# OSU-NLP-Group/saev

Hardware: AMD Instinct MI355X
Metric: activations/sec (train step), d_in=1024 x32 k=32 (higher is better)
Workload: dtype f32 (encoder: fp16 MFMA first pass with a rigorous error margin, survivors recomputed exactly in fp32; all else fp32)

## Files before the change

saev_amd/csrc/ctx_forward.hip:

```cpp
#include "ctx.h"

extern "C" {


int saev_normalize_w_dec(saev_ctx* c, void* stream) {
    if (!c) return SAEV_INVALID_ARG;
    REQUIRE(c, c->params, SAEV_NOT_BOUND, "parameters not bound");
    if (!c->cfg.normalize_w_dec) return SAEV_OK;
    HIPCHK(c, launch_normalize_rows(c->params + c->off_W_dec, c->cfg.d_sae, c->cfg.d_model, (hipStream_t)stream));
    return SAEV_OK;
}

static bool bind_x_sources(saev_ctx* c, const float* x, int n, bool allow_borrow) {
    saev_ctx* l = c->leader;
    const bool borrow = allow_borrow && l != nullptr && l->xprep_x == x && l->xprep_n == n && l->xprep_serial != c->leader_serial_seen;
    saev_ctx* src = borrow ? l : c;
    c->upper_c = src->upper; c->mu_c = src->mu; c->xnorm_c = src->xnorm; c->xabs_c = src->xabs_part; c->xs_c = src->xs;
    c->borrow_streamed = borrow && l->fwd_streamed && l->mu_keep != nullptr;
    if (c->borrow_streamed) c->mu_c = l->mu_keep;
    c->fwd_step = c->fwd_slices && (src == c || src->fwd_slices);
    c->xS_c = c->fwd_step ? src->xS : nullptr;
    if (borrow) c->leader_serial_seen = l->xprep_serial;
    return borrow;
}
// ... 86 lines not shown
        if (predicted) { a.heur_z = c->heur_state; a.tau_max = c->tau_max; }
        a.refresh_first = 8;
        a.refresh_every = a.ngroups > 32 ? 1 : 2;
        HIPCHK(c, launch_encode_f16x3(a, epi, s));
        return SAEV_OK;
    }
    EncodeArgs a{};
    a.x = x;
    a.W_enc = c->params + c->off_W_enc;
    a.b_enc = c->params + c->off_b_enc;
    a.n_rows = n;
    a.D = c->cfg.d_model;
    a.S = c->cfg.d_sae;
    a.s_splits = encoder_splits(n, a.S, encode_gemm_tile_rows(), encode_gemm_tile_latents(), 512);
    a.h_out = h_out;
    a.ngroups = c->cfg.top_k <= 32 ? 32 : 64;
    a.gmax = c->gmax;
    a.gmax_stride = c->gmax_stride;
    a.cand_cnt = c->cand_cnt;
    a.cand_val = c->cand_val;
    a.cand_idx = c->cand_idx;
    a.cand_cap = CAND_CAP; a.cand_stride = CAND_STRIDE;
    a.enable_flag = flag;
    a.enable_when = when;
    HIPCHK(c, launch_encode_gemm(a, epi, s));
    return SAEV_OK;
}

int saev_encode_dense(saev_ctx* c, const float* x, int32_t n, float* h_out, void* stream) {
    if (!c) return SAEV_INVALID_ARG;
    REQUIRE(c, c->params, SAEV_NOT_BOUND, "parameters not bound");
    REQUIRE(c, x && h_out && n > 0, SAEV_INVALID_ARG, "saev_encode_dense: bad arguments");
    REQUIRE(c, n <= c->cfg.max_batch || c->cfg.encoder_mode == SAEV_ENCODER_F32, SAEV_INVALID_ARG,
            "saev_encode_dense: n_rows > max_batch");
    bind_x_sources(c, x, n, false);
    c->xprep_x = nullptr;
    if (c->relu_train && c->cfg.encoder_mode == SAEV_ENCODER_F16X3) {
        hipStream_t s = (hipStream_t)stream;
        HIPCHK(c, hipMemsetAsync(c->rt_scales + 8, 0, sizeof(float), s));
        HIPCHK(c, launch_absmax(x, (long)n * c->cfg.d_model, c->rt_scales + 8, s));
        int rc = prepare_dense_scaled(c, x, n, c->rt_scales + 8, c->rt_scales + 10, s);
        if (rc != SAEV_OK) return rc;
        return run_encoder(c, x, n, EPI_DENSE, h_out, nullptr, 0, s, false, c->rt_scales + 10);
    }
    if (c->cfg.encoder_mode != SAEV_ENCODER_F16R) {
        int rc = prepare_encoder(c, x, n, nullptr, (hipStream_t)stream);
        if (rc != SAEV_OK) return rc;
    }
    return run_encoder(c, x, n, EPI_DENSE, h_out, nullptr, 0, (hipStream_t)stream);
}

int saev_topk_dense(saev_ctx* c, const float* h, int32_t n, int32_t k, const int32_t* mask, int32_t* idx_out,
                    float* val_out, void* stream) {
    if (!c) return SAEV_INVALID_ARG;
    REQUIRE(c, h && idx_out && val_out && n > 0 && k > 0, SAEV_INVALID_ARG, "saev_topk_dense: bad arguments");
    REQUIRE(c, k <= c->cfg.d_sae, SAEV_INVALID_ARG, "saev_topk_dense: k > d_sae");
    SelectDenseArgs a{};
    a.h = h; a.n_rows = n; a.S = c->cfg.d_sae; a.k = k; a.mask = mask;
    a.idx_out = idx_out; a.val_out = val_out; a.out_stride = k;
    HIPCHK(c, launch_select_dense(a, (hipStream_t)stream));
    return SAEV_OK;
}

static int encode_topk_impl(saev_ctx* c, const float* x, int n, int32_t* idx_out, float* val_out,
                            const int32_t* pre_flag, hipStream_t s, const float* xmax_dev = nullptr, bool x_borrowed = false) {
    const int K = c->cfg.top_k;
    int32_t* need_dense = c->flags + 1;
    const bool f16r_mode = c->cfg.encoder_mode == SAEV_ENCODER_F16R;
    const bool predict_mode = fused_supported(c->cfg) && c->cfg.bound_mode != 0 && c->cfg.encoder_mode != SAEV_ENCODER_F32 &&
                              f16_ngroups(c) == 32;
    const bool one_launch_pre = fused_supported(c->cfg) && !predict_mode;
    if (c->follow_stream) {
        HIPCHK(c, launch_follower_scales(c->leader->xside_keep, c->wmax_prev, scl(c), const_cast<int32_t*>(pre_flag), 1, s));
    } else if (!c->stream_step) {
        int rc0 = prepare_encoder(c, x, n, const_cast<int32_t*>(pre_flag), s, xmax_dev, x_borrowed, one_launch_pre);
        if (rc0 != SAEV_OK) return rc0;
        rc0 = wait_wenc(c, s);
        if (rc0 != SAEV_OK) return rc0;
    }
    if (fused_supported(c->cfg)) {
        const int ng = c->cfg.encoder_mode == SAEV_ENCODER_F32 ? (c->cfg.top_k <= 32 ? 32 : 64) : f16_ngroups(c);
        const bool f16r = c->cfg.encoder_mode == SAEV_ENCODER_F16R;
        auto select_stage = [&](const int32_t* flag, int when, int32_t* bad, const int32_t* tau_max, int32_t* ovf = nullptr,
                                const int32_t* first_flag = nullptr) -> int {
            SelectCandArgs sc{};
            sc.cand_cnt = c->cand_cnt; sc.cand_val = c->cand_val; sc.cand_idx = c->cand_idx;
            sc.cand_cap = CAND_CAP; sc.cand_stride = CAND_STRIDE; sc.n_rows = n; sc.k = K;
            sc.idx_out = idx_out; sc.val_out = val_out; sc.out_stride = K;
            sc.enable_flag = first_flag ? first_flag : flag; sc.enable_when = when;
            sc.tau_max = tau_max; sc.invalid = bad; sc.ovf = ovf;
            if (f16r) {
                sc.row_margin = c->row_margin; sc.x = x; sc.W_encT = c->dW_encT; sc.b_enc = c->params + c->off_b_enc;
                sc.D = c->cfg.d_model; sc.refine_overflow = bad;
                sc.surv_idx = c->surv_idx; sc.surv_val = c->surv_val; sc.surv_cnt = c->surv_cnt;
                if (c->fwd_step) { sc.surv_rng = c->surv_rng; sc.lat_range = c->rs_lat_range; sc.n_ranges = c->rs_n_ranges; }
                HIPCHK(c, launch_select_cand(sc, s));
                sc.enable_flag = flag; sc.ovf = nullptr;
                if (c->fwd_step) {
                    RefineSlicesArgs rs{};
                    rs.surv_idx = c->surv_idx; rs.surv_cnt = c->surv_cnt; rs.surv_val = c->surv_val; rs.surv_rng = c->surv_rng;
                    rs.xS = c->xS_c; rs.WeS = c->stream_ok ? c->WeS : c->dW_encT; rs.b_enc = sc.b_enc; rs.part = c->rs_part;
                    rs.n_rows = n; rs.S = c->cfg.d_sae; rs.D = c->cfg.d_model;
                    rs.lat_range = c->rs_lat_range; rs.n_ranges = c->rs_n_ranges;
                    rs.enable_flag = flag; rs.enable_when = when;
                    HIPCHK(c, launch_refine_slices(rs, s));
                    sc.sum_part = c->rs_part; sc.sum_bias = sc.b_enc; sc.sum_n = c->cfg.d_model / RS_SLICE; sc.sum_plane = (size_t)n * REFINE_CAP;
                } else {
                    HIPCHK(c, launch_refine_exact(sc, s));
                }
                sc.row_margin = nullptr; sc.tau_max = nullptr;
                sc.cand_cnt = c->surv_cnt; sc.cand_val = c->surv_val; sc.cand_idx = c->surv_idx; sc.cand_cap = REFINE_CAP; sc.cand_stride = REFINE_CAP;
            }
            HIPCHK(c, launch_select_cand(sc, s));
            return SAEV_OK;
        };
        const bool predict = c->cfg.bound_mode != 0 && ng == 32 && c->cfg.encoder_mode != SAEV_ENCODER_F32;
        int32_t *bad1 = c->flags + 9, *run2 = c->flags + 10, *gate = c->flags + 11;
        if (predict) {
            HIPCHK(c, launch_heur_gate(c->heur_state, pre_flag, gate, s));
            HIPCHK(c, launch_encoder_init(c->cand_cnt, n, c->gmax, 0, s, c->tau_max));
            timing_begin(c, s);
            int rc = run_encoder(c, x, n, EPI_TOPK, nullptr, gate, 0, s, true);
            if (rc != SAEV_OK) return rc;
            timing_end(c, s);
            HIPCHK(c, launch_overflow_check(c->cand_cnt, n, CAND_CAP, gate, bad1, c->flags + 2, c->flags + 3, s, need_dense,
                                            nullptr, c->heur_state + 3, nullptr, pre_flag));
            rc = select_stage(bad1, 0, bad1, c->tau_max);
            if (rc != SAEV_OK) return rc;
            HIPCHK(c, launch_heur_update(c->heur_state, bad1, c->heur_state + 3, K, gate, s));
            HIPCHK(c, launch_encoder_init(c->cand_cnt, n, c->gmax, ng * c->gmax_stride, s, nullptr, bad1, 1));
            rc = run_encoder(c, x, n, EPI_TOPK, nullptr, bad1, 1, s);
            if (rc != SAEV_OK) return rc;
            HIPCHK(c, launch_overflow_check(c->cand_cnt, n, CAND_CAP, pre_flag, need_dense, c->flags + 2, c->flags + 3, s, need_dense,
                                            run2, nullptr, bad1));
            rc = select_stage(run2, 1, need_dense, nullptr);
            if (rc != SAEV_OK) return rc;
        } else {
            const int S_ = c->cfg.d_sae;
            if (c->stream_step) {
                const int D_ = c->cfg.d_model;
                XprepArgs xp{};
                xp.x = c->gather_pool != nullptr ? c->gather_pool : x; xp.rows = c->gather_rows; xp.x_out = c->gather_pool != nullptr ? const_cast<float*>(x) : nullptr;
                xp.n = n; xp.D = D_; xp.nks = D_ / 32; xp.n_pad = c->MB_pad; xp.scales = scl(c); xp.mu = c->mu; xp.xs = c->xs; xp.xS = c->xS;
                xp.xn_part = c->xn_part; xp.col_part = c->colsum_partials; xp.amax_part = c->amax_part; xp.cmax_part = c->cmax_part;
                xp.W_enc = c->params + c->off_W_enc; xp.WeS = c->WeS; xp.b_enc = c->params + c->off_b_enc; xp.b_seen = c->b_seen;
                xp.S = S_; xp.salt = ++c->stale_salt; xp.stale = c->flags + 12;
                if (!c->followers.empty()) { xp.mu_keep = c->mu_keep; xp.xside_keep = c->xside_keep; }
                HIPCHK(c, launch_xprep(xp, s));
                PreEncode2Args pe{};
                pe.cand_cnt = c->cand_cnt; pe.n_rows = n; pe.gmax = c->gmax; pe.n_gmax = ng * c->gmax_stride;
                pe.xn_part = c->xn_part; pe.nks = D_ / 32; pe.n_pad = c->MB_pad; pe.D = D_;
                pe.wg_part = c->wnorm_scratch; pe.n_part = (S_ + 255) / 256; pe.scales = scl(c); pe.scales_next = scl_next(c);
                pe.pre_flag = const_cast<int32_t*>(pre_flag); pe.wmax_prev = c->wmax_prev; pe.margin = c->row_margin; pe.xnorm = c->xnorm;
                pe.flags1 = c->flags + 1; pe.col_part = c->colsum_partials; pe.n_rowblk = (n + 255) / 256; pe.mu = c->mu;
                pe.inv_n = 1.0f / (float)n; pe.update_mu = c->train_fused ? 1 : 0;
                pe.amax_part = c->amax_part; pe.cmax_part = c->cmax_part; pe.n_img = ((n + 255) / 256) * (D_ / 32);
                pe.upper = c->upper; pe.stats = c->stats; pe.stale = c->flags + 12; pe.stale_host = c->stale_dev;
                pe.xside_keep = c->followers.empty() ? nullptr : c->xside_keep;
                HIPCHK(c, launch_pre_encode2(pe, s));
                if (c->train_fused) c->mu_serial++;
            } else
            HIPCHK(c, launch_pre_encode(c->cand_cnt, n, c->gmax, ng * c->gmax_stride, f16r_mode ? c->xnorm_c : nullptr, c->cfg.d_model,
                                        c->wnorm_scratch, (S_ + 255) / 256, f16r_mode ? scl(c) : nullptr, const_cast<int32_t*>(pre_flag),
                                        c->wmax_prev, c->row_margin, c->flags + 1, s));
            timing_begin(c, s);
            int rc = run_encoder(c, x, n, EPI_TOPK, nullptr, pre_flag, 0, s);
            if (rc != SAEV_OK) return rc;
            timing_end(c, s);
            rc = select_stage(need_dense, 0, need_dense, nullptr, c->flags + 1, pre_flag);
            if (rc != SAEV_OK) return rc;
        }
    } else {
        HIPCHK(c, launch_init_i32(need_dense, 1, 1, s));
        HIPCHK(c, hipMemsetAsync(c->flags + 2, 0, 2 * sizeof(int32_t), s));
        timing_begin(c, s);
        timing_end(c, s);
    }
    int rc = run_encoder(c, x, n, EPI_DENSE, c->h_dense, need_dense, 1, s);
    if (rc != SAEV_OK) return rc;
    SelectDenseArgs sd{};
    sd.h = c->h_dense; sd.n_rows = n; sd.S = c->cfg.d_sae; sd.k = K;
    sd.idx_out = idx_out; sd.val_out = val_out; sd.out_stride = K;
    sd.enable_flag = need_dense; sd.enable_when = 1;
    if (fused_supported(c->cfg)) sd.walk_grid = 4 * 256;
    HIPCHK(c, launch_select_dense(sd, s));
    return SAEV_OK;
}

int saev_encode_topk(saev_ctx* c, const float* x, int32_t n, int32_t* idx_out, float* val_out, void* stream) {
    if (!c) return SAEV_INVALID_ARG;
    REQUIRE(c, c->cfg.activation == SAEV_ACT_TOPK, SAEV_UNSUPPORTED,
            "saev_encode_topk: a TopK context only (ReLU: saev_encode_relu, BatchTopK: saev_encode_batch_topk)");
    REQUIRE(c, c->params, SAEV_NOT_BOUND, "parameters not bound");
    REQUIRE(c, x && idx_out && val_out && n > 0 && n <= c->cfg.max_batch, SAEV_INVALID_ARG,
            "saev_encode_topk: bad arguments (n_rows must be in 1..max_batch)");
    hipStream_t s = (hipStream_t)stream;
    HIPCHK(c, hipMemsetAsync(c->flags, 0, sizeof(int32_t), s));
    bind_x_sources(c, x, n, false);
    c->xprep_x = nullptr;
    c->stream_step = false;
    c->follow_stream = false;
    return encode_topk_impl(c, x, n, idx_out, val_out, c->flags, s);
}

int saev_scatter_dense(saev_ctx* c, const int32_t* idx, const float* val, int32_t n, int32_t k, float* f_out,
                       void* stream) {
    if (!c) return SAEV_INVALID_ARG;
    REQUIRE(c, idx && val && f_out && n > 0 && k > 0, SAEV_INVALID_ARG, "saev_scatter_dense: bad arguments");
    HIPCHK(c, launch_scatter_dense(idx, val, n, k, k, c->cfg.d_sae, f_out, (hipStream_t)stream));
    return SAEV_OK;
// ... 308 lines not shown
```

saev_amd/csrc/kernels.h:

```cpp
#pragma once
#include <hip/hip_runtime.h>
#include <stdint.h>

#include <string>

#include "../../include/saev_amd.h"

enum { EPI_DENSE = 0, EPI_TOPK = 1 };

struct EncodeArgs {
    const float* x;
    const float* W_enc;
    const float* b_enc;
    int n_rows, D, S;
    int s_splits;
    float* h_out;
    int ngroups;
    int32_t* gmax;
    int gmax_stride;
    int32_t* cand_cnt;
    float* cand_val;
    int32_t* cand_idx;
    int cand_cap;
    int cand_stride;
    const int32_t* enable_flag;
    int enable_when;
};

size_t encode_gemm_smem_bytes();
hipError_t launch_encode_gemm(const EncodeArgs& a, int epi, hipStream_t stream);
int encode_gemm_tile_rows();
int encode_gemm_tile_latents();

struct SelectDenseArgs {
    const float* h;
    int n_rows, S;
    int k;
    const int32_t* k_dev;
    const int32_t* mask;
    int32_t* idx_out;
    float* val_out;
    int out_stride;
    const int32_t* enable_flag;
    int enable_when;
    int walk_grid;
};
hipError_t launch_select_dense(const SelectDenseArgs& a, hipStream_t stream);

struct SelectCandArgs {
    const int32_t* cand_cnt;
    const float* cand_val;
    const int32_t* cand_idx;
    int cand_cap, cand_stride, n_rows, k;
    int32_t* idx_out;
    float* val_out;
    int out_stride;
    const int32_t* enable_flag;
    int enable_when;
    const float* row_margin;
    const float* x;
    const float* W_encT;
    const float* b_enc;
    int D;
    int32_t* surv_idx;
    float* surv_val;
    int32_t* surv_cnt;
    int32_t* refine_overflow;
    const int32_t* tau_max;
    int32_t* invalid;
    int32_t* ovf;
    int32_t* surv_rng;
    int lat_range, n_ranges;
    const float* sum_part;
    const float* sum_bias;
    int sum_n;
    size_t sum_plane;
};
hipError_t launch_refine_exact(const SelectCandArgs& a, hipStream_t stream);
constexpr int REFINE_CAP = 512;
constexpr int RS_SLICE = 32;
constexpr int RS_ROWS_MAX = 8;
constexpr int RS_LAT_RANGE = 32768;
constexpr int RS_MAX_RANGES = 8;
struct RefineSlicesArgs {
    const int32_t* surv_idx; const int32_t* surv_cnt; float* surv_val; const int32_t* surv_rng;
    const float* xS; const float* WeS; const float* b_enc; float* part;
    int n_rows, S, D, lat_range, n_ranges;
    const int32_t* enable_flag; int enable_when;
};
hipError_t launch_refine_slices(const RefineSlicesArgs& a, hipStream_t stream);
hipError_t launch_select_cand(const SelectCandArgs& a, hipStream_t stream);
hipError_t launch_init_i32(int32_t* p, int32_t v, int n, hipStream_t stream);
hipError_t launch_encoder_init(int32_t* cand_cnt, int n_rows, int32_t* gmax, int n_gmax, hipStream_t stream,
                               int32_t* tau_max = nullptr, const int32_t* enable_flag = nullptr, int enable_when = 0);
hipError_t launch_pre_encode(int32_t* cand_cnt, int n_rows, int32_t* gmax, int n_gmax, const float* xnorm, int D,
                             const float* wg_part, int n_part, const float* scales, int32_t* pre_flag, float* wmax_prev,
                             float* margin, int32_t* flags1, hipStream_t stream);
hipError_t launch_heur_gate(float* state, const int32_t* pre_flag, int32_t* gate, hipStream_t stream);
hipError_t launch_heur_update(float* state, const int32_t* bad, const float* cand_mean, int k, const int32_t* gate,
                              hipStream_t stream);
hipError_t launch_step_zero(saev_step_stats* stats, float* upper, int32_t* flag0, hipStream_t stream);
hipError_t launch_wnorm_max(const float* W_encT, int S, int D, float* wg_scratch, float* wmax, hipStream_t stream);
hipError_t launch_f16r_scales(const float* xmax_part, int n_part, const float* wmax, float* scales, hipStream_t stream);
hipError_t launch_pow2_scale(const float* absmax, float* pair, hipStream_t stream);
hipError_t launch_center_stats(const float* x, const float* mu, int n, int D, float* xnorm, float* wg_absmax,
                               hipStream_t stream, const float* xmax = nullptr);
hipError_t launch_row_margins(const float* xnorm, int n, int D, const float* wg_part, int n_part, const float* scales,
                              int32_t* pre_flag, float* wmax_prev, float* margin, hipStream_t stream);
hipError_t launch_overflow_check(const int32_t* cand_cnt, int n_rows, int cap, const int32_t* pre_flag,
                                 int32_t* need_dense, int32_t* n_overflow, int32_t* cand_max, hipStream_t stream,
                                 int32_t* dense_out = nullptr, int32_t* run_out = nullptr, float* cand_mean = nullptr,
                                 const int32_t* enable_flag = nullptr, const int32_t* dense_src = nullptr);

struct __attribute__((aligned(8))) RowStats {
    float sse_scaled;
    float l0;
    float l1;
    float aux_sse;
    double sse64;
    double sumsq64;
};

struct DecodeArgs {
    const float* x;
    const int32_t* idx;
    const float* val;
    int code_stride, k;
    const float* W_dec;
    const float* b_dec;
    int n_rows, D, S;
    int idx_limit;
    const float* upper;
    float gscale;
    int training;
    float* g;
    float* x_hat;
    int32_t* fired;
    RowStats* rowstats;
    float* gS;
    float* xS;
    float* dval_out;
    uint32_t* csc_bitmap;
    int csc_words;
};
hipError_t launch_decode(const DecodeArgs& a, hipStream_t stream);
bool decode_forms_dval(int D, int k);
bool decode_matry_forms_dval(int D, int k);

constexpr int MAX_PREFIXES = 16;
struct MatryArgs {
    int P;
    int32_t cuts[MAX_PREFIXES];
    float* G;
    int g_rows_all;
};
hipError_t launch_decode_matry(const DecodeArgs& a, const MatryArgs& m, hipStream_t stream);

struct CscArgs {
    const int32_t* idx;
    int code_stride, k;
// ... 495 lines not shown
```

saev_amd/csrc/select.hip:

```cpp
#include "common.h"
#include "kernels.h"

namespace {

constexpr int SD_THREADS = 256;

__device__ __forceinline__ int block_excl_scan_256(int v, int* lds_wave_tot, int& total) {
    const int lane = threadIdx.x & 63, w = threadIdx.x >> 6;
    int incl = v;
#pragma unroll
    for (int o = 1; o < 64; o <<= 1) {
        int n = __shfl_up(incl, o, 64);
        if (lane >= o) incl += n;
    }
    if (lane == 63) lds_wave_tot[w] = incl;
    __syncthreads();
    int base = 0, tot = 0;
#pragma unroll
    for (int i = 0; i < 4; ++i) {
        const int t = lds_wave_tot[i];
        if (i < w) base += t;
        tot += t;
    }
    total = tot;
// ... 73 lines not shown
        int flg[4] = {0, 0, 0, 0}, feq[4] = {0, 0, 0, 0};
        if (q < S4) {
            v = *reinterpret_cast<const f32x4*>(h + 4 * q);
            int4 mk = {1, 1, 1, 1};
            if (a.mask) mk = *reinterpret_cast<const int4*>(a.mask + 4 * q);
            const int m[4] = {mk.x, mk.y, mk.z, mk.w};
#pragma unroll
            for (int e = 0; e < 4; ++e) {
                const uint32_t key = f2ukey(v[e]);
                flg[e] = (m[e] != 0 && key > T);
                feq[e] = (m[e] != 0 && key == T);
            }
        }
        const int ngt = flg[0] + flg[1] + flg[2] + flg[3];
        const int neq = feq[0] + feq[1] + feq[2] + feq[3];
        int tot;
        const int ex = block_excl_scan_256(ngt | (neq << 16), wave_tot, tot);
        int gt_before = base_gt + (ex & 0xFFFF);
        int eq_before = base_eq + (ex >> 16);
#pragma unroll
        for (int e = 0; e < 4; ++e) {
            if (flg[e]) {
                const int pos = gt_before + min(eq_before, need);
                oi[pos] = 4 * q + e;
                ov[pos] = v[e];
                ++gt_before;
            } else if (feq[e]) {
                if (eq_before < need) {
                    const int pos = gt_before + eq_before;
                    oi[pos] = 4 * q + e;
                    ov[pos] = v[e];
                }
                ++eq_before;
            }
        }
        base_gt += tot & 0xFFFF;
        base_eq += tot >> 16;
    }
    __syncthreads();
    }
}


__device__ __forceinline__ float wave_reduce_scatter8(float (&p)[8], int lane) {
    int bit = 32;
#pragma unroll
    for (int h = 4; h >= 1; h >>= 1, bit >>= 1) {
        const bool up = (lane & bit) != 0;
#pragma unroll
        for (int i = 0; i < h; ++i) {
            const float keep = up ? p[i + h] : p[i];
            const float send = up ? p[i] : p[i + h];
            p[i] = keep + __shfl_xor(send, bit, 64);
        }
    }
    float r = p[0];
    for (; bit >= 1; bit >>= 1) r += __shfl_xor(r, bit, 64);
    return r;
}

__device__ __forceinline__ void sort_by_idx_and_store(const SelectCandArgs& a, int row, int k, int32_t my_idx, float my_val,
                                                      int lane) {
#pragma unroll
    for (int size = 2; size <= 64; size <<= 1) {
#pragma unroll
        for (int stride = size >> 1; stride > 0; stride >>= 1) {
            const int32_t o_idx = __shfl_xor(my_idx, stride, 64);
            const float o_val = __shfl_xor(my_val, stride, 64);
            const bool up = ((lane & size) == 0);
            const bool lower = ((lane & stride) == 0);
            const bool take_other = (lower == up) ? (o_idx < my_idx) : (o_idx > my_idx);
            if (take_other) { my_idx = o_idx; my_val = o_val; }
        }
    }
    if (lane < a.k) {
        const bool ok = lane < k;
        a.idx_out[(size_t)row * a.out_stride + lane] = ok ? my_idx : -1;
        a.val_out[(size_t)row * a.out_stride + lane] = ok ? my_val : 0.f;
    }
}

template <int EPL>
__device__ __forceinline__ void select_cand_row(const SelectCandArgs& a, int row, int n, int32_t (&s_idx)[4][64],
                                                float (&s_val)[4][64], const float* cv, const int32_t* ci) {
    const int lane = threadIdx.x & 63;
    const int w = threadIdx.x >> 6;
    const int k = min(a.k, n);

    uint32_t key[EPL];
    int32_t idx[EPL];
#pragma unroll
    for (int e = 0; e < EPL; ++e) {
        const int p = e * 64 + lane;
        if (p < n) { key[e] = f2ukey(cv[p]); idx[e] = ci[p]; }
        else { key[e] = 0u; idx[e] = 0x7fffffff; }
    }
    auto kth_largest = [&]() {
        uint32_t t = 0;
        for (int bit = 31; bit >= 0; --bit) {
            const uint32_t trial = t | (1u << bit);
            int c = 0;
#pragma unroll
            for (int e = 0; e < EPL; ++e) c += __popcll(__ballot(key[e] >= trial));
            if (c == k) {
                uint32_t m = 0xffffffffu;
#pragma unroll
                for (int e = 0; e < EPL; ++e) m = min(m, key[e] >= trial ? key[e] : 0xffffffffu);
#pragma unroll
                for (int o = 32; o > 0; o >>= 1) m = min(m, (uint32_t)__shfl_xor((int)m, o, 64));
                return m;
            }
            if (c > k) t = trial;
        }
        return t;
    };
    uint32_t T = kth_largest();
    if (a.tau_max != nullptr && lane == 0 && (n < a.k || ukey2f(T) < key2f(a.tau_max[row]))) *a.invalid = 1;
    if (a.row_margin != nullptr) {
        const uint32_t key_lo = f2ukey(ukey2f(T) - a.row_margin[row]);
        int32_t* so = a.surv_idx + (size_t)row * REFINE_CAP;
        int base = 0;
        const int n_rng = a.surv_rng != nullptr ? a.n_ranges : 1;
        for (int r = 0; r < n_rng; ++r) {
            const int32_t lo = r * a.lat_range, hi = (r == n_rng - 1) ? 0x7ffffffe : lo + a.lat_range;
#pragma unroll
            for (int e = 0; e < EPL; ++e) {
                const bool sv = key[e] >= key_lo && idx[e] >= lo && idx[e] <= hi - (r == n_rng - 1 ? 0 : 1);
                const unsigned long long m = __ballot(sv);
                const int pos = base + __popcll(m & ((1ull << lane) - 1ull));
                if (sv && pos < REFINE_CAP) so[pos] = idx[e];
                base += __popcll(m);
            }
            if (a.surv_rng != nullptr && lane == 0) a.surv_rng[(size_t)row * RS_MAX_RANGES + r] = min(base, REFINE_CAP);
        }
        if (lane == 0) {
            a.surv_cnt[row] = min(base, REFINE_CAP);
            if (base > REFINE_CAP) *a.refine_overflow = 1;
        }
        return;
    }
    int cgt = 0, ceq = 0;
#pragma unroll
    for (int e = 0; e < EPL; ++e) { cgt += __popcll(__ballot(key[e] > T)); ceq += __popcll(__ballot(key[e] == T)); }
    const int need = k - cgt;
    int32_t idx_cut = 0x7fffffff;
    if (ceq > need) {
        int32_t X = 0;
        for (int bit = 30; bit >= 0; --bit) {
            const int32_t trial = X | (1 << bit);
            int c = 0;
#pragma unroll
            for (int e = 0; e < EPL; ++e) c += __popcll(__ballot(key[e] == T && idx[e] < trial));
            if (c < need) X = trial;
        }
        idx_cut = X;
    }
    s_idx[w][lane] = 0x7fffffff;
    s_val[w][lane] = 0.f;
    int base = 0;
#pragma unroll
    for (int e = 0; e < EPL; ++e) {
        const bool sel = (key[e] > T) || (key[e] == T && idx[e] <= idx_cut);
        const unsigned long long m = __ballot(sel);
        const int pos = base + __popcll(m & ((1ull << lane) - 1ull));
        if (sel && pos < 64) { s_idx[w][pos] = idx[e]; s_val[w][pos] = ukey2f(key[e]); }
        base += __popcll(m);
    }
    sort_by_idx_and_store(a, row, k, s_idx[w][lane], s_val[w][lane], lane);
}

__device__ __forceinline__ int stream_count(const float* cv, const int32_t* ci, int n, uint32_t lo_key, int mode, uint32_t T,
                                            int32_t idx_lt, int lane) {
    int c = 0;
    for (int p0 = 0; p0 < n; p0 += 64) {
        const int p = p0 + lane;
        bool hit = false;
        if (p < n) {
// ... 57 lines not shown
        }
        return;
    }
    const uint32_t T = stream_kth_largest(cv, ci, n, k, lane);
    if (a.tau_max != nullptr && lane == 0 && (n < a.k || ukey2f(T) < key2f(a.tau_max[row]))) *a.invalid = 1;
    const int cgt = stream_count(cv, ci, n, 0u, 1, T, 0, lane), ceq = stream_count(cv, ci, n, 0u, 2, T, 0, lane);
    const int need = k - cgt;
    int32_t idx_cut = 0x7fffffff;
    if (ceq > need) {
        int32_t X = 0;
        for (int bit = 30; bit >= 0; --bit) {
            const int32_t trial = X | (1 << bit);
            if (stream_count(cv, ci, n, 0u, 3, T, trial, lane) < need) X = trial;
        }
        idx_cut = X;
    }
    s_idx[w][lane] = 0x7fffffff;
    s_val[w][lane] = 0.f;
    int base = 0;
    for (int p0 = 0; p0 < n; p0 += 64) {
        const int p = p0 + lane;
        uint32_t key = 0u;
        int32_t idx = 0x7fffffff;
        if (p < n) { key = f2ukey(cv[p]); idx = ci[p]; }
        const bool sel = p < n && ((key > T) || (key == T && idx <= idx_cut));
        const unsigned long long m = __ballot(sel);
        const int pos = base + __popcll(m & ((1ull << lane) - 1ull));
        if (sel && pos < 64) { s_idx[w][pos] = idx; s_val[w][pos] = ukey2f(key); }
        base += __popcll(m);
    }
    sort_by_idx_and_store(a, row, k, s_idx[w][lane], s_val[w][lane], lane);
}

__device__ __forceinline__ void select_small_row(const SelectCandArgs& a, int row, int n, const float* cv, const int32_t* ci) {
    const int lane = threadIdx.x & 63;
    const int k = min(a.k, n);
    uint32_t key = 0u;
    int32_t idx = 0x7fffffff;
    if (lane < n) {
        key = f2ukey(cv[lane]);
        idx = ci[lane];
    }
#pragma unroll
    for (int size = 2; size <= 64; size <<= 1) {
#pragma unroll
        for (int stride = size >> 1; stride > 0; stride >>= 1) {
            const uint32_t o_key = __shfl_xor(key, stride, 64);
            const int32_t o_idx = __shfl_xor(idx, stride, 64);
            const bool other_first = (o_key > key) || (o_key == key && o_idx < idx);
            const bool up = ((lane & size) == 0);
            const bool lower = ((lane & stride) == 0);
            const bool take_other = (lower == up) ? other_first : !other_first;
            if (take_other) { key = o_key; idx = o_idx; }
        }
    }
    if (a.tau_max != nullptr) {
        const float kth = ukey2f(__shfl(key, max(k - 1, 0), 64));
        if (lane == 0 && (n < a.k || kth < key2f(a.tau_max[row]))) *a.invalid = 1;
    }
    const bool win = lane < k;
    sort_by_idx_and_store(a, row, k, win ? idx : 0x7fffffff, win ? ukey2f(key) : 0.f, lane);
}

template <bool BIG>
__global__ __launch_bounds__(256) void select_cand_kernel(SelectCandArgs a) {
    if (a.enable_flag != nullptr && (*a.enable_flag != 0) != (a.enable_when != 0)) return;
    __shared__ int32_t s_idx[4][64];
    __shared__ float s_val[4][64];
    const int row = blockIdx.x * 4 + (threadIdx.x >> 6);
    if (row >= a.n_rows) return;
    const int cnt = a.cand_cnt[row];
    if (a.ovf != nullptr && (threadIdx.x & 63) == 0 && cnt > a.cand_cap) atomicOr(&a.ovf[0], 1);
    if (a.ovf != nullptr && a.row_margin != nullptr && (threadIdx.x & 63) == 0 && !(a.row_margin[row] < 3.0e38f)) atomicOr(&a.ovf[0], 1);
    const int n = min(cnt, a.cand_cap);
    const float* cv = a.cand_val + (size_t)row * a.cand_stride;
    const int32_t* ci = a.cand_idx + (size_t)row * a.cand_stride;
    __shared__ float l_sum[4][REFINE_CAP];
    if (a.sum_part != nullptr) {
        float* const lv = l_sum[threadIdx.x >> 6];
        for (int j = threadIdx.x & 63; j < n; j += 64) {
            const size_t o = (size_t)row * a.cand_stride + j;
            float sv = 0.f;
            int c = 0;
            for (; c + 8 <= a.sum_n; c += 8) {
                float v[8];
#pragma unroll
                for (int u = 0; u < 8; ++u) v[u] = a.sum_part[(size_t)(c + u) * a.sum_plane + o];
#pragma unroll
                for (int u = 0; u < 8; ++u) sv += v[u];
            }
            for (; c < a.sum_n; ++c) sv += a.sum_part[(size_t)c * a.sum_plane + o];
            lv[j] = sv + a.sum_bias[ci[j]];
        }
        __asm__ volatile("" ::: "memory");
        cv = lv;
    }
    if (n <= 64 && a.row_margin == nullptr) select_small_row(a, row, n, cv, ci);
    else if (n <= 512) select_cand_row<8>(a, row, n, s_idx, s_val, cv, ci);
    else if (n <= 1024) select_cand_row<16>(a, row, n, s_idx, s_val, cv, ci);
    else if (n <= 2048) select_cand_row<32>(a, row, n, s_idx, s_val, cv, ci);
    else if constexpr (BIG) select_cand_row<64>(a, row, n, s_idx, s_val, cv, ci);
    else select_cand_row_stream(a, row, n, s_idx, s_val, cv, ci);
}

__global__ void init_i32_kernel(int32_t* p, int32_t v, int n) {
    const int i = blockIdx.x * blockDim.x + threadIdx.x;
    if (i < n) p[i] = v;
}

__global__ void encoder_init_kernel(int32_t* cand_cnt, int n_rows, int32_t* gmax, int n_gmax, int32_t* tau_max,
                                    const int32_t* enable_flag, int enable_when) {
    if (enable_flag != nullptr && (*enable_flag != 0) != (enable_when != 0)) return;
    const int i = blockIdx.x * blockDim.x + threadIdx.x;
    if (i < n_rows) cand_cnt[i] = 0;
    if (i < n_gmax) gmax[i] = INT32_MIN;
    if (tau_max != nullptr && i < n_rows) tau_max[i] = INT32_MIN;
}
__global__ void step_zero_kernel(saev_step_stats* stats, float* upper, int32_t* flag0) {
    if (threadIdx.x == 0) {
        *stats = saev_step_stats{};
        *upper = 0.f;
        *flag0 = 0;
    }
}

template <int NV>
__global__ __launch_bounds__(256) void refine_exact_kernel(SelectCandArgs a) {
    if (a.enable_flag != nullptr && (*a.enable_flag != 0) != (a.enable_when != 0)) return;
    const int lane = threadIdx.x & 63;
    const int row = blockIdx.x * 4 + (threadIdx.x >> 6);
    if (row >= a.n_rows) return;
    const int ns = a.surv_cnt[row];
    const int D4 = a.D >> 2;
    f32x4 xv[NV];
    const f32x4* xr = reinterpret_cast<const f32x4*>(a.x + (size_t)row * a.D);
#pragma unroll
    for (int n = 0; n < NV; ++n) xv[n] = (lane + 64 * n < D4) ? xr[lane + 64 * n] : f32x4{0.f, 0.f, 0.f, 0.f};
    const int32_t* si = a.surv_idx + (size_t)row * REFINE_CAP;
    float* sv = a.surv_val + (size_t)row * REFINE_CAP;
    for (int j0 = 0; j0 < ns; j0 += 8) {
        const int32_t my = si[min(j0 + (lane & 7), ns - 1)];
        float p[8];
#pragma unroll
        for (int t = 0; t < 8; ++t) {
            const int32_t li = __shfl(my, t, 64);
            const f32x4* wr = reinterpret_cast<const f32x4*>(a.W_encT + (size_t)li * a.D);
            float acc = 0.f;
#pragma unroll
            for (int n = 0; n < NV; ++n) {
                if (lane + 64 * n < D4) {
                    const f32x4 wv = wr[lane + 64 * n];
                    acc += xv[n][0] * wv[0] + xv[n][1] * wv[1] + xv[n][2] * wv[2] + xv[n][3] * wv[3];
                }
            }
            p[t] = acc;
        }
        const float r = wave_reduce_scatter8(p, lane);
        if ((lane & 7) == 0) {
            const int t = lane >> 3;
            if (j0 + t < ns) sv[j0 + t] = r + a.b_enc[si[j0 + t]];
        }
    }
}

typedef int i32x4 __attribute__((ext_vector_type(4)));
__device__ __forceinline__ f32x4 rs_buf_load16(__amdgpu_buffer_rsrc_t r, uint32_t voff) {
    const i32x4 v = __builtin_amdgcn_raw_buffer_load_b128(r, voff, 0, 0);
    return f32x4{__int_as_float(v[0]), __int_as_float(v[1]), __int_as_float(v[2]), __int_as_float(v[3])};
}
__device__ __forceinline__ float group8_reduce_scatter(float (&p)[8], int li) {
    {
        const bool up = (li & 4) != 0;
#pragma unroll
        for (int i = 0; i < 4; ++i) {
            const float keep = up ? p[i + 4] : p[i], send = up ? p[i] : p[i + 4];
            p[i] = keep + __shfl_xor(send, 4, 64);
        }
    }
    {
        const bool up = (li & 2) != 0;
#pragma unroll
        for (int i = 0; i < 2; ++i) {
            const float keep = up ? p[i + 2] : p[i], send = up ? p[i] : p[i + 2];
            p[i] = keep + __shfl_xor(send, 2, 64);
// ... 316 lines not shown
    float m = 0.f;
    for (int i = threadIdx.x; i < n_part; i += 256) m = fmaxf(m, xmax_part[i]);
    m = wave_max(m);
    if ((threadIdx.x & 63) == 0) sh[threadIdx.x >> 6] = m;
    __syncthreads();
    if (threadIdx.x == 0) {
        const float xm = fmaxf(fmaxf(sh[0], sh[1]), fmaxf(sh[2], sh[3])), wm = *wmax;
        scales[0] = (xm > 0.f && xm < 3.0e38f) ? exp2f(13.0f - floorf(log2f(xm))) : 1.0f;
        scales[1] = (wm > 0.f && wm < 3.0e38f) ? exp2f(13.0f - floorf(log2f(wm))) : 1.0f;
        scales[2] = scales[0];
        scales[3] = 1.0f;
    }
}

__global__ void overflow_check_kernel(const int32_t* cand_cnt, int n_rows, int cap, const int32_t* pre_flag,
                                      int32_t* bad_out, int32_t* n_overflow, int32_t* cand_max, int32_t* dense_out,
                                      int32_t* run_out, float* cand_mean, const int32_t* enable_flag,
                                      const int32_t* dense_src) {
    if (enable_flag != nullptr && *enable_flag == 0) {
        if (threadIdx.x == 0 && run_out != nullptr) *run_out = 0;
        return;
    }
    __shared__ int sh, shmax, shsum;
    if (threadIdx.x == 0) { sh = 0; shmax = 0; shsum = 0; }
    __syncthreads();
    int c = 0, m = 0, t = 0;
    for (int i = threadIdx.x; i < n_rows; i += blockDim.x) { const int v = cand_cnt[i]; c += (v > cap); m = max(m, v); t += min(v, cap); }
    c = wave_sum_i(c);
    t = wave_sum_i(t);
#pragma unroll
    for (int o = 32; o > 0; o >>= 1) m = max(m, __shfl_xor(m, o, 64));
    if ((threadIdx.x & 63) == 0) { if (c) atomicAdd(&sh, c); atomicMax(&shmax, m); atomicAdd(&shsum, t); }
    __syncthreads();
    if (threadIdx.x == 0) {
        const int pre = (pre_flag && *pre_flag) ? 1 : 0;
        *n_overflow = sh;
        *cand_max = shmax;
        if (cand_mean != nullptr) *cand_mean = (float)shsum / (float)max(n_rows, 1);
        if (run_out == nullptr) {
            *bad_out = (pre || sh > 0) ? 1 : 0;
            if (dense_out != nullptr) *dense_out = dense_src != nullptr ? (*dense_src != 0 ? 1 : 0) : pre;
        } else {
            const int dense = (*dense_out != 0 || sh > 0) ? 1 : 0;
            *dense_out = dense;
            *run_out = dense ? 0 : 1;
        }
    }
}

__global__ void heur_gate_kernel(float* state, const int32_t* pre_flag, int32_t* gate) {
    if (threadIdx.x != 0) return;
    int g = (pre_flag != nullptr && *pre_flag != 0) ? 1 : 0;
    if (state[5] > 0.f) { state[5] -= 1.f; g = 1; }
    *gate = g;
}
__global__ void heur_update_kernel(float* state, const int32_t* bad, const float* cand_mean, int k, const int32_t* gate) {
    if (threadIdx.x != 0 || *gate != 0) return;
    float z = state[0];
    state[2] += 1.f;
    if (*bad != 0) {
        z -= 0.3f;
        state[1] += 1.f;
        state[4] += 1.f;
        if (state[4] >= 3.f) { state[4] = 0.f; state[5] = 256.f; z = 1.5f; }
    } else {
        state[4] = 0.f;
        if (*cand_mean > 3.f * (float)k) z += 0.002f;
    }
    state[0] = fminf(fmaxf(z, 0.5f), 3.5f);
}

}

hipError_t launch_select_dense(const SelectDenseArgs& a, hipStream_t stream) {
    if (a.n_rows <= 0) return hipSuccess;
    const int grid = (a.walk_grid > 0 && a.walk_grid < a.n_rows) ? a.walk_grid : a.n_rows;
    hipLaunchKernelGGL(select_dense_kernel, dim3(grid), dim3(SD_THREADS), 0, stream, a);
    return hipGetLastError();
}

hipError_t launch_select_cand(const SelectCandArgs& a, hipStream_t stream) {
    if (a.n_rows <= 0) return hipSuccess;
    if (a.cand_cap > 4096 || (a.sum_part != nullptr && a.cand_cap > REFINE_CAP)) return hipErrorInvalidValue;
    if (a.k > 32) hipLaunchKernelGGL(select_cand_kernel<true>, dim3((a.n_rows + 3) / 4), dim3(256), 0, stream, a);
    else hipLaunchKernelGGL(select_cand_kernel<false>, dim3((a.n_rows + 3) / 4), dim3(256), 0, stream, a);
    return hipGetLastError();
}

hipError_t launch_init_i32(int32_t* p, int32_t v, int n, hipStream_t stream) {
    if (n <= 0) return hipSuccess;
    hipLaunchKernelGGL(init_i32_kernel, dim3((n + 255) / 256), dim3(256), 0, stream, p, v, n);
    return hipGetLastError();
}

hipError_t launch_encoder_init(int32_t* cand_cnt, int n_rows, int32_t* gmax, int n_gmax, hipStream_t stream, int32_t* tau_max,
                               const int32_t* enable_flag, int enable_when) {
    const int n = n_rows > n_gmax ? n_rows : n_gmax;
    if (n <= 0) return hipSuccess;
    hipLaunchKernelGGL(encoder_init_kernel, dim3((n + 255) / 256), dim3(256), 0, stream, cand_cnt, n_rows, gmax, n_gmax, tau_max,
                       enable_flag, enable_when);
    return hipGetLastError();
}
hipError_t launch_pre_encode(int32_t* cand_cnt, int n_rows, int32_t* gmax, int n_gmax, const float* xnorm, int D,
                             const float* wg_part, int n_part, const float* scales, int32_t* pre_flag, float* wmax_prev,
                             float* margin, int32_t* flags1, hipStream_t stream) {
    const int n = std::max(1, n_rows > n_gmax ? n_rows : n_gmax);
    hipLaunchKernelGGL(pre_encode_kernel, dim3((n + 255) / 256), dim3(256), 0, stream, cand_cnt, n_rows, gmax, n_gmax, xnorm, D,
                       wg_part, n_part, scales, pre_flag, wmax_prev, margin, flags1);
    return hipGetLastError();
}
hipError_t launch_follower_scales(const float* xside, const float* wmax, float* scales, int32_t* pre_flag, int keep_w, hipStream_t stream) {
    hipLaunchKernelGGL(follower_scales_kernel, dim3(1), dim3(64), 0, stream, xside, wmax, scales, pre_flag, keep_w);
    return hipGetLastError();
}
hipError_t launch_pre_encode2(PreEncode2Args a, hipStream_t stream) {
    a.nb_rows = (std::max(1, std::max(a.n_rows, a.n_gmax)) + 255) / 256;
    hipLaunchKernelGGL(pre_encode2_kernel, dim3(a.nb_rows + (a.D + 255) / 256), dim3(256), 0, stream, a);
    return hipGetLastError();
}
hipError_t launch_heur_gate(float* state, const int32_t* pre_flag, int32_t* gate, hipStream_t stream) {
    hipLaunchKernelGGL(heur_gate_kernel, dim3(1), dim3(64), 0, stream, state, pre_flag, gate);
    return hipGetLastError();
}
hipError_t launch_heur_update(float* state, const int32_t* bad, const float* cand_mean, int k, const int32_t* gate,
                              hipStream_t stream) {
    hipLaunchKernelGGL(heur_update_kernel, dim3(1), dim3(64), 0, stream, state, bad, cand_mean, k, gate);
    return hipGetLastError();
}
hipError_t launch_step_zero(saev_step_stats* stats, float* upper, int32_t* flag0, hipStream_t stream) {
    hipLaunchKernelGGL(step_zero_kernel, dim3(1), dim3(64), 0, stream, stats, upper, flag0);
    return hipGetLastError();
}

hipError_t launch_wnorm_max(const float* W_encT, int S, int D, float* wg_scratch, float* wmax, hipStream_t stream) {
    const int nwg = (S + 3) / 4;
    hipLaunchKernelGGL(rownorm_wgmax_kernel, dim3(nwg), dim3(256), 0, stream, W_encT, S, D, wg_scratch);
    hipLaunchKernelGGL(max_reduce_kernel, dim3(1), dim3(1024), 0, stream, wg_scratch, nwg, wmax);
    return hipGetLastError();
}
hipError_t launch_f16r_scales(const float* xmax_part, int n_part, const float* wmax, float* scales, hipStream_t stream) {
    hipLaunchKernelGGL(f16r_scales_kernel, dim3(1), dim3(256), 0, stream, xmax_part, n_part, wmax, scales);
    return hipGetLastError();
}
hipError_t launch_pow2_scale(const float* absmax, float* pair, hipStream_t stream) {
    hipLaunchKernelGGL(pow2_scale_kernel, dim3(1), dim3(64), 0, stream, absmax, pair);
    return hipGetLastError();
}
hipError_t launch_center_stats(const float* x, const float* mu, int n, int D, float* xnorm, float* wg_absmax,
                               hipStream_t stream, const float* xmax) {
    hipLaunchKernelGGL(center_stats_kernel, dim3((n + 3) / 4), dim3(256), 0, stream, x, mu, n, D, xnorm, wg_absmax, xmax);
    return hipGetLastError();
}
hipError_t launch_max_reduce(const float* v, int n, float* out, hipStream_t stream) {
    hipLaunchKernelGGL(max_reduce_kernel, dim3(1), dim3(1024), 0, stream, v, n, out);
    return hipGetLastError();
}
hipError_t launch_row_margins(const float* xnorm, int n, int D, const float* wg_part, int n_part, const float* scales,
                              int32_t* pre_flag, float* wmax_prev, float* margin, hipStream_t stream) {
    hipLaunchKernelGGL(row_margin_kernel, dim3((n + 255) / 256), dim3(256), 0, stream, xnorm, n, D, wg_part, n_part, scales,
                       pre_flag, wmax_prev, margin);
    return hipGetLastError();
}

hipError_t launch_refine_exact(const SelectCandArgs& a, hipStream_t stream) {
    if (a.n_rows <= 0) return hipSuccess;
    const dim3 grid((a.n_rows + 3) / 4), block(256);
    const int nv = (a.D / 4 + 63) / 64;
// ... 29 lines not shown
```

Measured before the change: 6.209 million.

## Prefilter top-k candidates using per-group max lower bound before selection

Adds a select_pre_kernel that takes the k-th largest of the per-group maxima as a lower bound on the row's top-k threshold, minus the fp16 row margin when one is set. It compacts only candidates above that bound into a small shared position list before running the radix-style selection, and falls back to the full stream path when the bound is unusable or the list overflows. The aim is to shrink the per-row sort/select work over large candidate lists. It also widens the refine partial-sum reduction to 32-wide unrolled loads. This costs an extra candidate pass and more shared memory per block, and the first predict-stage selection is excluded.

```diff
diff --git a/saev_amd/csrc/ctx_forward.hip b/saev_amd/csrc/ctx_forward.hip
--- a/saev_amd/csrc/ctx_forward.hip
+++ b/saev_amd/csrc/ctx_forward.hip
@@ -192,13 +192,14 @@
         const int ng = c->cfg.encoder_mode == SAEV_ENCODER_F32 ? (c->cfg.top_k <= 32 ? 32 : 64) : f16_ngroups(c);
         const bool f16r = c->cfg.encoder_mode == SAEV_ENCODER_F16R;
         auto select_stage = [&](const int32_t* flag, int when, int32_t* bad, const int32_t* tau_max, int32_t* ovf = nullptr,
-                                const int32_t* first_flag = nullptr) -> int {
+                                const int32_t* first_flag = nullptr, bool bounded = true) -> int {
             SelectCandArgs sc{};
             sc.cand_cnt = c->cand_cnt; sc.cand_val = c->cand_val; sc.cand_idx = c->cand_idx;
             sc.cand_cap = CAND_CAP; sc.cand_stride = CAND_STRIDE; sc.n_rows = n; sc.k = K;
             sc.idx_out = idx_out; sc.val_out = val_out; sc.out_stride = K;
             sc.enable_flag = first_flag ? first_flag : flag; sc.enable_when = when;
             sc.tau_max = tau_max; sc.invalid = bad; sc.ovf = ovf;
+            if (bounded) { sc.gmax = c->gmax; sc.gmax_stride = c->gmax_stride; sc.gmax_groups = ng; }
             if (f16r) {
                 sc.row_margin = c->row_margin; sc.x = x; sc.W_encT = c->dW_encT; sc.b_enc = c->params + c->off_b_enc;
                 sc.D = c->cfg.d_model; sc.refine_overflow = bad;
@@ -218,7 +219,7 @@
                 } else {
                     HIPCHK(c, launch_refine_exact(sc, s));
                 }
-                sc.row_margin = nullptr; sc.tau_max = nullptr;
+                sc.row_margin = nullptr; sc.tau_max = nullptr; sc.gmax = nullptr;
                 sc.cand_cnt = c->surv_cnt; sc.cand_val = c->surv_val; sc.cand_idx = c->surv_idx; sc.cand_cap = REFINE_CAP; sc.cand_stride = REFINE_CAP;
             }
             HIPCHK(c, launch_select_cand(sc, s));
@@ -235,7 +236,7 @@
             timing_end(c, s);
             HIPCHK(c, launch_overflow_check(c->cand_cnt, n, CAND_CAP, gate, bad1, c->flags + 2, c->flags + 3, s, need_dense,
                                             nullptr, c->heur_state + 3, nullptr, pre_flag));
-            rc = select_stage(bad1, 0, bad1, c->tau_max);
+            rc = select_stage(bad1, 0, bad1, c->tau_max, nullptr, nullptr, false);
             if (rc != SAEV_OK) return rc;
             HIPCHK(c, launch_heur_update(c->heur_state, bad1, c->heur_state + 3, K, gate, s));
             HIPCHK(c, launch_encoder_init(c->cand_cnt, n, c->gmax, ng * c->gmax_stride, s, nullptr, bad1, 1));
diff --git a/saev_amd/csrc/kernels.h b/saev_amd/csrc/kernels.h
--- a/saev_amd/csrc/kernels.h
+++ b/saev_amd/csrc/kernels.h
@@ -75,7 +75,10 @@
     const float* sum_bias;
     int sum_n;
     size_t sum_plane;
-};
+    const int32_t* gmax;
+    int gmax_stride, gmax_groups;
+};
+constexpr int SC_PRE_CAP = 1024;
 hipError_t launch_refine_exact(const SelectCandArgs& a, hipStream_t stream);
 constexpr int REFINE_CAP = 512;
 constexpr int RS_SLICE = 32;
diff --git a/saev_amd/csrc/select.hip b/saev_amd/csrc/select.hip
--- a/saev_amd/csrc/select.hip
+++ b/saev_amd/csrc/select.hip
@@ -179,7 +179,8 @@
 
 template <int EPL>
 __device__ __forceinline__ void select_cand_row(const SelectCandArgs& a, int row, int n, int32_t (&s_idx)[4][64],
-                                                float (&s_val)[4][64], const float* cv, const int32_t* ci) {
+                                                float (&s_val)[4][64], const float* cv, const int32_t* ci,
+                                                const uint16_t* pos = nullptr) {
     const int lane = threadIdx.x & 63;
     const int w = threadIdx.x >> 6;
     const int k = min(a.k, n);
@@ -189,7 +190,7 @@
 #pragma unroll
     for (int e = 0; e < EPL; ++e) {
         const int p = e * 64 + lane;
-        if (p < n) { key[e] = f2ukey(cv[p]); idx[e] = ci[p]; }
+        if (p < n) { const int q = pos != nullptr ? (int)pos[p] : p; key[e] = f2ukey(cv[q]); idx[e] = ci[q]; }
         else { key[e] = 0u; idx[e] = 0x7fffffff; }
     }
     auto kth_largest = [&]() {
@@ -413,6 +414,13 @@
             const size_t o = (size_t)row * a.cand_stride + j;
             float sv = 0.f;
             int c = 0;
+            for (; c + 32 <= a.sum_n; c += 32) {
+                float v[32];
+#pragma unroll
+                for (int u = 0; u < 32; ++u) v[u] = a.sum_part[(size_t)(c + u) * a.sum_plane + o];
+#pragma unroll
+                for (int u = 0; u < 32; ++u) sv += v[u];
+            }
             for (; c + 8 <= a.sum_n; c += 8) {
                 float v[8];
 #pragma unroll
@@ -431,6 +439,75 @@
     else if (n <= 1024) select_cand_row<16>(a, row, n, s_idx, s_val, cv, ci);
     else if (n <= 2048) select_cand_row<32>(a, row, n, s_idx, s_val, cv, ci);
     else if constexpr (BIG) select_cand_row<64>(a, row, n, s_idx, s_val, cv, ci);
+    else select_cand_row_stream(a, row, n, s_idx, s_val, cv, ci);
+}
+
+__global__ __launch_bounds__(256, 8) void select_pre_kernel(SelectCandArgs a) {
+    if (a.enable_flag != nullptr && (*a.enable_flag != 0) != (a.enable_when != 0)) return;
+    __shared__ int32_t s_idx[4][64];
+    __shared__ float s_val[4][64];
+    __shared__ uint16_t l_pos[4][SC_PRE_CAP];
+    const int lane = threadIdx.x & 63, w = threadIdx.x >> 6;
+    const int row = blockIdx.x * 4 + w;
+    if (row >= a.n_rows) return;
+    const float* cv = a.cand_val + (size_t)row * a.cand_stride;
+    const int32_t* ci = a.cand_idx + (size_t)row * a.cand_stride;
+    const int cnt = a.cand_cnt[row];
+    const int ng = a.gmax_groups, kk = min(a.k, ng);
+    uint32_t u = kk == ng ? 0xffffffffu : 0u;
+    if (lane < ng) u = (uint32_t)a.gmax[(size_t)lane * a.gmax_stride + row] ^ 0x80000000u;
+    const float margin = a.row_margin != nullptr ? a.row_margin[row] : 0.f;
+    float v[8];
+#pragma unroll
+    for (int t = 0; t < 8; ++t) v[t] = cv[64 * t + lane];
+    if (a.ovf != nullptr && lane == 0 && cnt > a.cand_cap) atomicOr(&a.ovf[0], 1);
+    if (a.ovf != nullptr && a.row_margin != nullptr && lane == 0 && !(margin < 3.0e38f)) atomicOr(&a.ovf[0], 1);
+    const int n = min(cnt, a.cand_cap);
+    uint32_t key_L = 0;
+    if (kk == ng) {
+        key_L = u;
+#pragma unroll
+        for (int o = 32; o > 0; o >>= 1) key_L = min(key_L, (uint32_t)__shfl_xor((int)key_L, o, 64));
+    } else {
+        for (int bit = 31; bit >= 0; --bit) {
+            const uint32_t trial = key_L | (1u << bit);
+            if (__popcll(__ballot(u >= trial)) >= kk) key_L = trial;
+        }
+    }
+    const float L = ukey2f(key_L);
+    const float lo = a.row_margin != nullptr ? L - margin : L;
+    bool usable = fabsf(L) <= 3.0e38f && lo <= L;
+    const uint32_t key_lo = a.row_margin != nullptr ? f2ukey(lo) : key_L;
+    int m = 0, c_L = 0;
+    if (usable) {
+        for (int p0 = 0; p0 < n; p0 += 512) {
+            if (p0 > 0) {
+#pragma unroll
+                for (int t = 0; t < 8; ++t) {
+                    const int p = p0 + 64 * t + lane;
+                    v[t] = p < n ? cv[p] : 0.f;
+                }
+            }
+#pragma unroll
+            for (int t = 0; t < 8; ++t) {
+                const int p = p0 + 64 * t + lane;
+                const uint32_t key = p < n ? f2ukey(v[t]) : 0u;
+                const bool hit = key >= key_lo;
+                const unsigned long long hm = __ballot(hit);
+                const int pos = m + __popcll(hm & ((1ull << lane) - 1ull));
+                if (hit && pos < SC_PRE_CAP) l_pos[w][pos] = (uint16_t)p;
+                m += __popcll(hm);
+                c_L += __popcll(__ballot(key >= key_L));
+            }
+        }
+        usable = c_L >= a.k && m <= SC_PRE_CAP;
+    }
+    __asm__ volatile("" ::: "memory");
+    if (usable) {
+        if (m <= 256) select_cand_row<4>(a, row, m, s_idx, s_val, cv, ci, l_pos[w]);
+        else if (m <= 512) select_cand_row<8>(a, row, m, s_idx, s_val, cv, ci, l_pos[w]);
+        else select_cand_row<16>(a, row, m, s_idx, s_val, cv, ci, l_pos[w]);
+    } else if (n <= 64 && a.row_margin == nullptr) select_small_row(a, row, n, cv, ci);
     else select_cand_row_stream(a, row, n, s_idx, s_val, cv, ci);
 }
 
@@ -913,7 +990,9 @@
 hipError_t launch_select_cand(const SelectCandArgs& a, hipStream_t stream) {
     if (a.n_rows <= 0) return hipSuccess;
     if (a.cand_cap > 4096 || (a.sum_part != nullptr && a.cand_cap > REFINE_CAP)) return hipErrorInvalidValue;
-    if (a.k > 32) hipLaunchKernelGGL(select_cand_kernel<true>, dim3((a.n_rows + 3) / 4), dim3(256), 0, stream, a);
+    if (a.gmax != nullptr && a.sum_part == nullptr && a.k <= 32 && a.cand_stride >= 512 && a.cand_cap <= 65536)
+        hipLaunchKernelGGL(select_pre_kernel, dim3((a.n_rows + 3) / 4), dim3(256), 0, stream, a);
+    else if (a.k > 32) hipLaunchKernelGGL(select_cand_kernel<true>, dim3((a.n_rows + 3) / 4), dim3(256), 0, stream, a);
     else hipLaunchKernelGGL(select_cand_kernel<false>, dim3((a.n_rows + 3) / 4), dim3(256), 0, stream, a);
     return hipGetLastError();
 }
```

Measured after the change: 6.266 million, median of 6. No clear change (+0.9%).
